# madsjulia/GeostatInversion.jl

Hardware: AMD Instinct MI355X
Metric: randSVD GB/s + top-k singular-value rel-err, n=1e6 rank=256 (higher is better)
Workload: dtype f64

## Files before the change

### geostatinversion.jl_amd/build.py

```python
import os
import shutil
import subprocess
import sys
from concurrent.futures import ThreadPoolExecutor

HERE = os.path.dirname(os.path.abspath(__file__))
CSRC = os.path.join(HERE, "csrc")
OBJ = os.path.join(HERE, "build")
LIB = os.path.join(HERE, "libgsi_hip.so")
SOURCES = ["gemm_f64.hip", "gemm_f64_gen1.hip", "syrk_f64.hip", "panel_lu_leaf.hip", "panel_lu_blocks.hip", "panel_lu_streamed.hip", "panel_lu_sharded.hip", "panel_qr.hip", "cholqr.hip", "lowrank_power.hip", "jacobi_svd.hip", "misc.hip", "lsqr_dev.hip", "pointcov_gemm.hip", "fft_cov.hip", "fft_gridcov_plan.hip", "fftrf_sample.hip",
           "hip_backend.hip", "pipeline.cpp", "api.cpp"]
HEADERS = ["backend.hpp", "hip_common.hpp", "panel_lu_dev.hpp", "pipeline.hpp", "lsqr_state.hpp", "pointcov.hpp", "pointcov_gen.hpp", "host_staging.hpp", "gemm_f64_kernel.inc.hpp", "fft_line.hpp", "jacobi_sched.hpp", "../../include/gsi_hip.h"]
CXXFLAGS = ["-O3", "-std=c++17", "-fPIC", "--offload-arch=gfx950", "-Wall", "-Wno-unused-function",
            "-Wno-unused-result", "-Wno-unused-value"]
RESOURCE_FLAG = "-Rpass-analysis=kernel-resource-usage"
_RES_KEYS = {"TotalSGPRs": "sgprs", "VGPRs": "vgprs", "AGPRs": "agprs", "ScratchSize [bytes/lane]": "scratch_bytes_per_lane",
             "Occupancy [waves/SIMD]": "occupancy_waves_per_simd", "SGPRs Spill": "sgpr_spills", "VGPRs Spill": "vgpr_spills",
             "LDS Size [bytes/block]": "lds_bytes_per_block", "Dynamic Stack": "dynamic_stack"}


def parse_resource_remarks(text):
    out, cur = {}, None
    for line in text.splitlines():
        if "remark:" not in line or "[-Rpass-analysis=kernel-resource-usage]" not in line:
            continue
        body = line.split("remark:", 1)[1].replace("[-Rpass-analysis=kernel-resource-usage]", "").strip()
        if ":" not in body:
            continue
        key, val = [x.strip() for x in body.rsplit(":", 1)]
        if key == "Function Name":
            cur = out.setdefault(val, {})
        elif cur is not None and key in _RES_KEYS:
            cur[_RES_KEYS[key]] = (val == "True") if key == "Dynamic Stack" else int(val)
    return out


def hipcc_version():
    r = subprocess.run([_hipcc(), "--version"], capture_output=True, text=True)
    lines = [ln.strip() for ln in r.stdout.splitlines() if ln.strip()]
    return "; ".join(lines[:2])


def kernel_resources():
# ... 74 lines not shown
```

### geostatinversion.jl_amd/context.py

```python
import ctypes as C

import numpy as np

from . import _lib as L


class Context:

    def __init__(self, device=0, lib=None):
        self.lib = lib or L.load()
        h = C.c_void_p()
        L.check(self.lib.gsi_ctx_create(C.byref(h), int(device)), self.lib)
        self.h = h
        self.device = int(device)
        self._children = []

    def close(self):
        if getattr(self, "h", None):
            for ch in list(self._children):
                ch.close()
            self.lib.gsi_ctx_destroy(self.h)
            self.h = None

    def __del__(self):
# ... 24 lines not shown
        out = np.empty((self.rank()[1], v.size))
        L.check(self.lib.gsi_ctx_host_allgather(self.h, L.dptr(v), v.size, L.dptr(out)), self.lib)
        return out

    def barrier(self):
        self.host_allgather([0.0])

    def shard(self, m):
        r, n = self.rank()
        pad = -(-m // n)
        row0 = min(r * pad, m)
        return row0, min(pad, m - row0)

    def profile(self, on=True):
        L.check(self.lib.gsi_ctx_profile(self.h, int(on)), self.lib)

    def phase_reset(self):
        L.check(self.lib.gsi_ctx_phase_reset(self.h), self.lib)

    def phase_times(self):
        ms = (C.c_double * len(L.PHASES))()
        cnt = (C.c_int64 * len(L.PHASES))()
        L.check(self.lib.gsi_ctx_phase_times(self.h, ms, cnt), self.lib)
        return {name: (ms[i], cnt[i]) for i, name in enumerate(L.PHASES)}

    def counters(self):
        out = (C.c_int64 * 4)()
        L.check(self.lib.gsi_ctx_counters(self.h, out), self.lib)
        return {"cholqr2": out[0], "householder": out[1], "jacobi_sweeps": out[2], "scholqr3": out[3]}

    LU_FORMS = ["none", "replicated", "per-step", "persistent-1hop", "persistent-2hop", "persistent-ov"]

    def path_info(self):
        n = 18
        out = (C.c_int64 * n)()
        L.check(self.lib.gsi_ctx_path_info(self.h, out, n), self.lib)
        forms = {self.LU_FORMS[f]: int(out[6 + f]) for f in range(1, 6) if out[6 + f]}
        return {"lu_form": self.LU_FORMS[out[0]] if 0 <= out[0] < 6 else int(out[0]), "lu_forms_run": forms,
                "lu_selftest_mask": int(out[1]), "collectives": int(out[2]), "n_ranks_seen": int(out[3]),
                "lu_timeouts": int(out[4]), "lu_timeouts_recovered": int(out[5]), "svd_sweep_cap_hits": int(out[12]),
                "lowrank_tails": int(out[13]), "lowrank_power_steps": int(out[14]), "lowrank_power_declines": int(out[15]),
                "lowrank_split_lus": int(out[16]), "lowrank_split_declines": int(out[17])}

    def release_cache(self):
        L.check(self.lib.gsi_ctx_release_cache(self.h), self.lib)

    def device_bytes(self):
        b = C.c_int64()
        L.check(self.lib.gsi_ctx_device_bytes(self.h, C.byref(b)), self.lib)
        return b.value


class _Handle:
    _destroy = None

    def __init__(self, ctx, h):
        self.ctx, self.h = ctx, h
        ctx._children.append(self)

    def close(self):
        if getattr(self, "h", None):
            getattr(self.ctx.lib, self._destroy)(self.h)
            self.h = None
            if self in self.ctx._children:
                self.ctx._children.remove(self)

    def __del__(self):
        try:
            self.close()
        except Exception:
            pass


class Operator(_Handle):
    _destroy = "gsi_op_destroy"
# ... 162 lines not shown
```

### geostatinversion.jl_amd/csrc/api.cpp

```cpp
#include <cmath>
#include <cstdlib>
#include <cstring>
#include <memory>
#include <new>
#include <string>
#include <vector>
#include "../../include/gsi_hip.h"
#include "pipeline.hpp"
#include "pointcov.hpp"

using namespace gsi;

struct gsi_ctx {
  Context c;
};
struct gsi_op {
  Operator op;
};
struct gsi_mat {
  gsi_ctx* ctx;
  Buf buf;
  int64_t rows, cols;
  int refs = 1;
};
// ... 135 lines not shown
    c.be->sync();
    if (!c.comm) {
      std::memcpy(all_out, mine, sizeof(double) * (size_t)count);
      return;
    }
    const int G = c.nranks();
    Buf send(c.be.get(), (size_t)count), recv(c.be.get(), (size_t)count * G);
    c.be->upload2d(send.p, count, mine, count, count, 1);
    const int64_t before = c.comm->ncollectives;
    c.comm->allgather(send.p, recv.p, (size_t)count);
    c.comm->ncollectives = before;
    c.be->download2d(all_out, count, recv.p, count, count, G);
  });
}

int gsi_ctx_path_info(gsi_ctx* ctx, int64_t* out, int64_t n_out) {
  return guarded([&] {
    REQUIRE(ctx && out && n_out >= 1, "bad argument");
    Context& c = ctx->c;
    int64_t v[GSI_PATH_INFO_COUNT] = {0};
    v[GSI_PATH_LU_FORM_LAST] = c.lu_form_last;
    v[GSI_PATH_LU_SELFTEST_MASK] = c.lus_mr_selftest;
    v[GSI_PATH_COLLECTIVES] = c.comm ? c.comm->ncollectives : 0;
    v[GSI_PATH_RANKS_SEEN] = c.ranks_seen;
    v[GSI_PATH_LU_TIMEOUTS] = c.be->lu_timeouts();
    v[GSI_PATH_LU_TIMEOUTS_RECOVERED] = c.lu_timeouts_recovered;
    for (int f = 0; f < (int)Context::LU_FORMS; ++f) v[GSI_PATH_LU_FORM_COUNTS + f] = c.lu_form_count[f];
    v[GSI_PATH_SVD_CAP_HITS] = c.be->svd_cap_hits();
    v[GSI_PATH_LOWRANK_TAILS] = c.lowrank_tails;
    v[GSI_PATH_LOWRANK_POWER_STEPS] = c.lowrank_power_steps;
    v[GSI_PATH_LOWRANK_POWER_DECLINES] = c.lowrank_power_declines;
    v[GSI_PATH_LOWRANK_SPLIT_LUS] = c.lowrank_split_lus;
    v[GSI_PATH_LOWRANK_SPLIT_DECLINES] = c.lowrank_split_declines;
    for (int64_t i = 0; i < n_out; ++i) out[i] = i < GSI_PATH_INFO_COUNT ? v[i] : 0;
  });
}

int gsi_ctx_pinned_copy_rate(gsi_ctx* ctx, int64_t bytes, double* h2d_gbs, double* d2h_gbs) {
  return guarded([&] {
    REQUIRE(ctx && h2d_gbs && d2h_gbs, "NULL argument");
    REQUIRE(bytes >= 0 && bytes <= ((int64_t)64 << 30), "bad size");
    ctx->c.be->pinned_copy_rate(bytes, h2d_gbs, d2h_gbs);
  });
}

int gsi_ctx_rank(gsi_ctx* ctx, int* rank, int* nranks) {
  return guarded([&] {
    REQUIRE(ctx, "ctx is NULL");
    if (rank) *rank = ctx->c.rank();
    if (nranks) *nranks = ctx->c.nranks();
  });
}

int gsi_op_dense(gsi_ctx* ctx, gsi_op** op, const double* A_rows, int64_t m, int64_t n, int64_t lda,
                 int64_t row0, int64_t m_local) {
  return guarded([&] {
    REQUIRE(ctx && op && A_rows, "NULL argument");
    *op = nullptr;
    REQUIRE(m >= 1 && n >= 1 && lda >= m_local && lda >= 1, "bad matrix shape");
    check_shard(ctx->c, m, row0, m_local);
    std::unique_ptr<gsi_op> o(new gsi_op());
    Operator& A = o->op;
    A.ctx = &ctx->c; A.kind = OP_DENSE; A.m = m; A.n = n; A.row0 = row0; A.mloc = m_local;
    A.ld = m_local > 0 ? ((m_local + 15) / 16) * 16 : 16;
    A.data = Buf(ctx->c.be.get(), (size_t)A.ld * n);
    ctx->c.be->upload2d(A.data.p, A.ld, A_rows, lda, m_local, n);
// ... 1035 lines not shown
```

### geostatinversion.jl_amd/csrc/backend.hpp

```cpp
#pragma once
#include <cstddef>
#include <cstdint>
#include <stdexcept>
#include <string>

namespace gsi {

struct Error : std::runtime_error {
  int code;
  Error(int c, const std::string& msg) : std::runtime_error(msg), code(c) {}
};

enum Phase : int {
  PH_GEMM_N = 0, PH_GEMM_T = 1, PH_LU = 2, PH_QR = 3, PH_SVD = 4, PH_SMALL_GEMM = 5,
  PH_COMM = 6, PH_OTHER = 7, PH_COMM_WAIT = 8, PH_COUNT = 9
};

class Backend {
 public:
  virtual ~Backend() {}
  virtual const char* name() const = 0;

  virtual double* alloc(size_t count) = 0;
  virtual void release(double* p) = 0;
// ... 153 lines not shown
                           double* out) = 0;

  virtual void gemv_n(int64_t m, int64_t k, double alpha, const double* A, int64_t lda, const double* x, double beta,
                      double* y) = 0;
  virtual void gemv_t(int64_t m, int64_t k, double alpha, const double* A, int64_t lda, const double* x, double* y) = 0;
  virtual void project_out(int64_t m, int64_t ncols, const double* q, double* Y, int64_t ld) = 0;
  virtual void scal(int64_t n, double a, double* x) = 0;
  virtual void diag_mul_add(int64_t n, const double* d, const double* x, double* y) = 0;

  virtual size_t lsqr_work_doubles() = 0;
  virtual void lsqr_begin(int64_t n, const double* w, double* work) = 0;
  virtual void lsqr_step_u(int64_t m, const double* t, double* u, double* work) = 0;
  virtual void lsqr_step_v(int64_t n, const double* t, double* v, double* w, double* x, double* work) = 0;

  virtual void f64_to_f32(const double* src, void* dst32, size_t count) = 0;
  virtual void pcga_params_f32(const void* Z32, int64_t n, int64_t K, const double* s, const double* X, double delta,
                               double* out) = 0;
  virtual void basis_gemv_f32(const void* Z32, int64_t n, int64_t K, const double* w, double beta, const double* X,
                              double* y) = 0;

  virtual int take_error(std::string* msg) = 0;
  virtual bool retryable_failure() { return false; }
  virtual void forgive_lost_coresidency() {}

  virtual void profile(bool on) = 0;
  virtual void phase_begin(Phase p) = 0;
  virtual void phase_end(Phase p) = 0;
  virtual void phase_end_more(Phase p) { phase_end(p); }
  virtual void phase_reset() = 0;
  virtual void phase_times(double* ms, int64_t* counts) = 0;
  virtual void counters(int64_t* out4) { out4[0] = out4[1] = out4[2] = out4[3] = 0; }
  virtual int64_t lu_timeouts() { return 0; }
  virtual int64_t svd_cap_hits() { return 0; }
  virtual void set_ranks_sharing_device(int n) { (void)n; }
};

class Comm {
 public:
  int rank = 0, nranks = 1;
  int64_t ncollectives = 0;
  virtual ~Comm() {}
  void allreduce_sum(double* buf, size_t count) { ++ncollectives; do_allreduce_sum(buf, count); }
  void allgather(const double* send, double* recv, size_t count) { ++ncollectives; do_allgather(send, recv, count); }
  void reduce_scatter_sum(const double* send, double* recv, size_t count) { ++ncollectives; do_reduce_scatter_sum(send, recv, count); }
  void alltoall(const double* send, double* recv, size_t count) { ++ncollectives; do_alltoall(send, recv, count); }
  virtual bool share_pointers(void* mine, size_t bytes, void** all) { (void)mine; (void)bytes; (void)all; return false; }
  virtual int ranks_on_my_device() { return 1; }
  virtual void host_barrier() {}

 protected:
  virtual void do_allreduce_sum(double* buf, size_t count) = 0;
  virtual void do_allgather(const double* send, double* recv, size_t count) = 0;
  virtual void do_reduce_scatter_sum(const double* send, double* recv, size_t count) = 0;
  virtual void do_alltoall(const double* send, double* recv, size_t count) = 0;
};

Backend* make_backend(int device_id);
Comm* make_comm(Backend* be, int nranks, int rank, const void* unique_id);
void comm_unique_id(void* id_out);
const char* backend_name();

struct ScopedPhase {
  Backend* be; Phase p;
  ScopedPhase(Backend* b, Phase ph) : be(b), p(ph) { be->phase_begin(p); }
  ~ScopedPhase() { be->phase_end(p); }
};
// ... 8 lines not shown
```

### geostatinversion.jl_amd/csrc/gemm_f64.hip

```cpp
#include <hip/hip_runtime.h>
#include <cstdint>
#include <cstdlib>
#include <type_traits>
#include <algorithm>
#include "hip_common.hpp"
#include "pointcov.hpp"
#include "pointcov_gen.hpp"

namespace gsi { namespace hipk {

#define GSI_GEMM_TILE_COUNTERS_32 1
#include "gemm_f64_kernel.inc.hpp"
void gemm_dispatch_gen1(int nt, dim3 grid, hipStream_t st, int64_t M, int64_t L, int64_t K, const double* A, int64_t lda,
                        const double* B, int64_t ldb, double* C, int64_t ldc, double alpha, double beta, double* slabs,
                        int64_t kchunk, int nchunks_x, int wide, int xmode, int tri, const GenA& gen, int64_t nitems);

__global__ void splitk_reduce_kernel(int64_t M, int64_t L, int nsplit, const double* __restrict__ slabs,
                                     double* __restrict__ C, int64_t ldc, double alpha, double beta) {
  const int64_t total = M * L;
  for (int64_t idx = (int64_t)blockIdx.x * blockDim.x + threadIdx.x; idx < total;
       idx += (int64_t)gridDim.x * blockDim.x) {
    double s = 0.0;
    for (int sp = 0; sp < nsplit; ++sp) s += slabs[(int64_t)sp * total + idx];
    const int64_t r = idx % M, c = idx / M;
    double v = alpha * s;
    if (beta != 0.0) v += beta * C[r + c * ldc];
    C[r + c * ldc] = v;
  }
}

int gemm_choose_split(int64_t nwg, int64_t K) {
  constexpr int64_t CUS = 256;
  static const bool legacy = getenv("GSI_GEMM_SPLIT_LEGACY") != nullptr;
  static const int forced = getenv("GSI_GEMM_FORCE_SPLIT") ? atoi(getenv("GSI_GEMM_FORCE_SPLIT")) : 0;
  if (forced > 0 && nwg >= 256 && K >= 64 * BK) return forced;
  if (legacy) {
    if (nwg >= 192 || K < 8 * BK) return 1;
    int64_t want = (CUS + nwg - 1) / nwg, cap = K / (4 * BK);
    if (want > cap) want = cap;
    return (int)(want < 1 ? 1 : (want > 64 ? 64 : want));
  }
  if (K < 8 * BK || nwg >= 16 * CUS) return 1;
  int64_t maxs = K / (4 * BK);
  if (maxs > 256) maxs = 256;
  int best = 1;
  double best_cost = (double)((nwg + CUS - 1) / CUS);
  for (int64_t s = 2; s <= maxs; ++s) {
    const double cost = (double)((nwg * s + CUS - 1) / CUS) / (double)s * (1.0 + 0.004 * (double)s);
// ... 34 lines not shown
  const int ntmax = gemm_chunk_tiles(tri);
  const int64_t nchunks = (tiles + ntmax - 1) / ntmax;
  const int nt = (int)((tiles + nchunks - 1) / nchunks);
  const int64_t rowblocks = (M + BMT - 1) / BMT;
  int64_t active = rowblocks * nchunks;
  if (tri == 1) {
    active = 0;
    for (int64_t rb = 0; rb < rowblocks; ++rb)
      for (int64_t cb = 0; cb < nchunks; ++cb)
        if (cb >= (rb * BMT) / ((int64_t)nt * 16)) ++active;
  }
  const int nsplit = (force_nsplit > 0) ? force_nsplit : ((K > 0) ? gemm_choose_split(active, K) : 1);
  int64_t kchunk = (K + nsplit - 1) / nsplit;
  kchunk = ((kchunk + BK - 1) / BK) * BK;
  if (kchunk == 0) kchunk = BK;
  const int ns_eff = (K > 0) ? (int)((K + kchunk - 1) / kchunk) : 1;
  dim3 grid((unsigned)active, (unsigned)ns_eff, 1);
  double* slabs = (ns_eff > 1) ? ws : nullptr;
  static const int ncus = [] { int dev = 0, n = 256; hipDeviceProp_t pr; if (hipGetDevice(&dev) == hipSuccess && hipGetDeviceProperties(&pr, dev) == hipSuccess) n = pr.multiProcessorCount; return n; }();
  static const bool persist_on = !(getenv("GSI_GEMM_PERSIST") != nullptr && getenv("GSI_GEMM_PERSIST")[0] == '0');
  int64_t nitems = 0;
  const bool a_ok = ((uintptr_t)A & 15) == 0 && (lda & 1) == 0;
  const bool b_ok = ((uintptr_t)B & 15) == 0 && (ldb & 1) == 0;
  const bool irregular_x = a_ok && (!b_ok || L % ((int64_t)nt * 16) != 0);
  const int wide = a_ok ? 1 : 0;
  const int xmode = big ? 2 : (irregular_x ? 1 : 0);
  if (persist_on && gen == nullptr && xmode == 0 && tri == 0 && ns_eff == 1 && (ncus & 7) == 0 && active >= 2 * (int64_t)ncus &&
      K <= 128 * BK) {
    nitems = active;
    grid.x = (unsigned)ncus;
  }
  if (plan != nullptr) *plan = {nt, nchunks, xmode, wide, ns_eff, nitems > 0 ? 1 : 0, (int64_t)grid.x, active};
  const GenA none = {nullptr, 1, 0, 0, 0, 0.0, 0.0, 0.0};
  if (gen != nullptr && gen_mode == 2)
    launch_dispatch<false, 2>(nt, grid, st, M, L, K, A, lda, B, ldb, C, ldc, alpha, beta, slabs, kchunk, (int)nchunks, wide, xmode, tri, *gen, nitems);
  else if (gen != nullptr)
    gemm_dispatch_gen1(nt, grid, st, M, L, K, A, lda, B, ldb, C, ldc, alpha, beta, slabs, kchunk, (int)nchunks, wide, xmode, tri, *gen, nitems);
  else if (transA)
    launch_dispatch<true, 0>(nt, grid, st, M, L, K, A, lda, B, ldb, C, ldc, alpha, beta, slabs, kchunk, (int)nchunks, wide, xmode, tri, none, nitems);
  else
    launch_dispatch<false, 0>(nt, grid, st, M, L, K, A, lda, B, ldb, C, ldc, alpha, beta, slabs, kchunk, (int)nchunks, wide, xmode, tri, none, nitems);
  if (ns_eff > 1) {
    const int64_t total = M * L;
    int blocks = (int)((total + 255) / 256);
    if (blocks > 2048) blocks = 2048;
    hipLaunchKernelGGL(splitk_reduce_kernel, dim3(blocks), dim3(256), 0, st, M, L, ns_eff, slabs, C, ldc,
                       alpha, beta);
  }
}

void gemm_splitk_reduce(hipStream_t st, int64_t M, int64_t L, int nsplit, const double* slabs, double* C, int64_t ldc) {
  const int64_t total = M * L;
  int blocks = (int)((total + 255) / 256);
  if (blocks > 2048) blocks = 2048;
  hipLaunchKernelGGL(splitk_reduce_kernel, dim3(blocks), dim3(256), 0, st, M, L, nsplit, slabs, C, ldc, 1.0, 0.0);
}

void gemm_f64(hipStream_t st, bool transA, int64_t M, int64_t L, int64_t K, double alpha, const double* A,
              int64_t lda, const double* B, int64_t ldb, double beta, double* C, int64_t ldc, double* ws, GemmPlan* plan) {
  gemm_launch(st, transA, nullptr, M, L, K, alpha, A, lda, B, ldb, beta, C, ldc, ws, 0, 1, 0, plan);
}

int gemm_split_for(int64_t M, int64_t L, int64_t K) {
  if (M <= 0 || L <= 0 || K <= 0) return 1;
  const int64_t tiles = (L + 15) / 16, nchunks = (tiles + NTMAX - 1) / NTMAX;
  const int64_t active = ((M + BMT - 1) / BMT) * nchunks;
// ... 53 lines not shown
```

### geostatinversion.jl_amd/csrc/gemm_f64_kernel.inc.hpp

```cpp
typedef double double4_t __attribute__((ext_vector_type(4)));

constexpr int MT = 2;
constexpr int BMT = 4 * 16 * MT;
constexpr int NTHREADS = 512;
constexpr int BK = 32;
constexpr int BKP = BK + 2;
constexpr int BMP = BMT + 16;
constexpr int NTMAX = 10;
constexpr int NSETS = 2;
constexpr int A_PAIRS = BMT * BK / (2 * NTHREADS);
constexpr int KSTEP_NN = 2 * NTHREADS / BMT;
constexpr int RSTEP = 2 * NTHREADS / BK;
static_assert(A_PAIRS * 2 * NTHREADS == BMT * BK, "tile does not divide over the threads");

struct GenA {
  const double* t2;
  int32_t ny;
  int32_t kind;
  int64_t roff;
  int64_t koff;
  double inv_ell2, sigma2, nugget;
  int32_t dim;
};

template <int NT, bool TRANS_A, int GEN, int XMODE>
__global__ __launch_bounds__(NTHREADS) void gemm_f64_kernel(
    int64_t M, int64_t L, int64_t K, const double* __restrict__ A, int64_t lda,
    const double* __restrict__ B, int64_t ldb, double* __restrict__ C, int64_t ldc, double alpha,
    double beta, double* __restrict__ slabs, int64_t kchunk, int nchunks_x, int wide, int tri, GenA gen, int64_t nitems) {
  static_assert(!(GEN != 0 && TRANS_A), "the generated operand is symmetric: only the NN form exists");
  constexpr bool CANP = (GEN == 0 && XMODE == 0);
  const bool persist = CANP && nitems > 0;
  constexpr bool RAGGED = XMODE != 0;
  constexpr bool BIG = XMODE == 2;
  using off_t = typename std::conditional<BIG, uint64_t, uint32_t>::type;
  constexpr int A_ELEMS = TRANS_A ? BMT * BKP : BK * BMP;
  constexpr int B_ELEMS = NT * 16 * BKP;
  constexpr int BUF_ELEMS = A_ELEMS + B_ELEMS;
  extern __shared__ double smem[];
  constexpr int LDS0 = (GEN == 2) ? 64 : 0;

  const int tid = threadIdx.x;
  const int lane = tid & 63;
  const int wave = tid >> 6;
  const int rg = wave & 3;
  const int ch = wave >> 2;
  constexpr int NTW = (NT + 1) / 2;
  const int jl = lane & 15;
  const int kk = lane >> 4;
  int64_t tile_lin = blockIdx.x;
  int split = (int)blockIdx.y;
  int64_t r0 = 0, c0 = 0;
  auto locate = [&](int64_t bx) __attribute__((always_inline)) {
    tile_lin = bx;
    const int T = (int)gridDim.x, S = (int)gridDim.y;
    if (S > 1 && (S & 7) == 0) {
      const int lin = (int)bx + T * (int)blockIdx.y;
      const int xcd = lin & 7, j = lin >> 3;
      split = xcd + 8 * (j / T);
      tile_lin = j % T;
    } else if (S == 1 && tri != 1 && nchunks_x > 1) {
      const int C8 = 8 * nchunks_x;
      const int nrb = (int)((M + BMT - 1) / BMT);
// ... 161 lines not shown
        }
        return;
      }
#pragma unroll
      for (int it = 0; it < B_PAIRS; ++it)
        if (!B_RAGGED || b_c + RSTEP * it < NT * 16)
          b_reg[set][it] = *reinterpret_cast<const double2*>(Bb + (b_off0 + (off_t)it * b_step));
      return;
    }
    if constexpr (GEN == 0) {
#pragma unroll
    for (int it = 0; it < A_PAIRS; ++it) {
      const char* p = Ab + (a_off0 + (off_t)it * a_step);
      const int64_t r = TRANS_A ? r0 + a_r + RSTEP * it : r0 + a_r;
      const int64_t k = TRANS_A ? k0 + a_k : k0 + a_k + KSTEP_NN * it;
      const bool ok0 = (r < M && k < kend);
      const bool ok1 = TRANS_A ? (r < M && k + 1 < kend) : (r + 1 < M && k < kend);
      a_reg[set][it].x = ok0 ? *reinterpret_cast<const double*>(p) : 0.0;
      a_reg[set][it].y = ok1 ? *reinterpret_cast<const double*>(p + 8) : 0.0;
    }
    }
#pragma unroll
    for (int it = 0; it < B_PAIRS; ++it) {
      const char* p = Bb + (b_off0 + (off_t)it * b_step);
      const int cl = b_c + RSTEP * it;
      const int64_t c = c0 + cl;
      const int64_t k = k0 + b_k;
      const bool okc = (cl < NT * 16) && (c < L);
      b_reg[set][it].x = (okc && k < kend) ? *reinterpret_cast<const double*>(p) : 0.0;
      b_reg[set][it].y = (okc && k + 1 < kend) ? *reinterpret_cast<const double*>(p + 8) : 0.0;
    }
  };

  auto stage = [&](int buf, auto SET, int64_t k0) __attribute__((always_inline)) {
    constexpr int set = decltype(SET)::value;
    double* a_s = smem + LDS0 + buf * BUF_ELEMS;
    double* b_s = a_s + A_ELEMS;
    (void)k0;
    if constexpr (GEN == 2) {
      const int kw = __builtin_amdgcn_readfirstlane(a_k);
      const int64_t row_first = gen.roff + r0;
      const int krem = (kend - k0 < BK) ? (int)(kend - k0) : BK;
#pragma unroll
      for (int it = 0; it < A_PAIRS; ++it) {
        const int64_t kc = k0 + kw + KSTEP_NN * it;
        const bool okk = kw + KSTEP_NN * it < krem;
        const int64_t gj = gen.koff + (okk ? kc : kbeg);
        const int64_t gju = ((int64_t)__builtin_amdgcn_readfirstlane((int)(gj >> 32)) << 32) |
                            (uint32_t)__builtin_amdgcn_readfirstlane((int)(gj & 0xffffffff));
        const double qx = A[4 * gju], qy = A[4 * gju + 1];
        double dx = p0x - qx, dy = p0y - qy;
        double s0 = fma(dx, dx, dy * dy);
        dx = p1x - qx; dy = p1y - qy;
        double s1 = fma(dx, dx, dy * dy);
        const int fl = gen_flags(gq.flags);
        if (fl & 1) {
          const double qz = A[4 * gju + 2];
          const double dz0 = p0z - qz, dz1 = p1z - qz;
          s0 = fma(dz0, dz0, s0); s1 = fma(dz1, dz1, s1);
        }
        double2 pr;
        gen_point_pair(gq, fl, s0, s1, gtab, pr.x, pr.y);
        const int rel = (int)(gju - row_first);
        if ((unsigned)rel < (unsigned)BMT) {
          pr.x += (a_r == rel) ? gen.nugget : 0.0;
          pr.y += (a_r + 1 == rel) ? gen.nugget : 0.0;
        }
        *reinterpret_cast<double2*>(a_s + (a_k + KSTEP_NN * it) * BMP + a_r) = pr;
      }
    } else
    if (TRANS_A) {
#pragma unroll
      for (int it = 0; it < A_PAIRS; ++it)
        *reinterpret_cast<double2*>(a_s + (a_r + RSTEP * it) * BKP + a_k) = a_reg[set][it];
    } else {
#pragma unroll
      for (int it = 0; it < A_PAIRS; ++it)
        *reinterpret_cast<double2*>(a_s + (a_k + KSTEP_NN * it) * BMP + a_r) = a_reg[set][it];
    }
#pragma unroll
    for (int it = 0; it < B_PAIRS; ++it)
      if (!B_RAGGED || b_c + RSTEP * it < NT * 16)
        *reinterpret_cast<double2*>(b_s + (b_c + RSTEP * it) * BKP + b_k) = b_reg[set][it];
  };

  double fa[MT], fan[MT];
  double fb[NTW];
  const int t0 = ch * NTW;
  const int ntw = (NT - t0 < NTW) ? ((NT - t0 > 0) ? NT - t0 : 0) : NTW;
  auto a_frag = [&](int buf, int s, int h) -> double {
    const double* a_s = smem + LDS0 + buf * BUF_ELEMS;
    return TRANS_A ? a_s[(16 * MT * rg + 16 * h + jl) * BKP + 4 * s + kk]
                   : a_s[(4 * s + kk) * BMP + 16 * MT * rg + 16 * h + jl];
  };
  auto b_frag = [&](int buf, int s, int t) -> double {
    const double* b_s = smem + LDS0 + buf * BUF_ELEMS + A_ELEMS;
    return b_s[(16 * (t0 + t) + jl) * BKP + 4 * s + kk];
  };

  using Set0 = std::integral_constant<int, 0>;
  using Set1 = std::integral_constant<int, 1>;
#if GSI_GEMM_TILE_COUNTERS_32
  auto do_tile = [&](int t, auto PAR) __attribute__((always_inline)) {
#else
  auto do_tile = [&](int64_t t, auto PAR) __attribute__((always_inline)) {
#endif
    constexpr int cur = decltype(PAR)::value;
    using NextSet = std::integral_constant<int, (NSETS == 2) ? (cur ^ 1) : 0>;
    auto chores = [&]() __attribute__((always_inline)) {
      __builtin_amdgcn_s_setprio(0);
#if GSI_GEMM_TILE_COUNTERS_32
      if (t + 1 < ntiles) stage(cur ^ 1, NextSet{}, kbeg + (int64_t)(t + 1) * BK);
      if (t + 1 + NSETS < ntiles) prefetch(t + 1 + NSETS, NextSet{});
#else
      if (t + 1 < ntiles) stage(cur ^ 1, NextSet{}, kbeg + (t + 1) * BK);
      if (t + 1 + NSETS < ntiles) prefetch(kbeg + (t + 1 + NSETS) * BK, NextSet{});
#endif
      __builtin_amdgcn_s_setprio(1);
    };
#pragma unroll
    for (int s = 0; s < BK / 4; ++s) {
      if (s == 1 && ch == 0) chores();
      if (s == 1 + BK / 8 && ch != 0) chores();
      const bool last = (s + 1 == BK / 4);
      if (last) __syncthreads();
      const int nbuf = last ? (cur ^ 1) : cur;
      const int ns = last ? 0 : s + 1;
      const bool more = !last || (t + 1 < ntiles);
      if (more) {
#pragma unroll
        for (int h = 0; h < MT; ++h) fan[h] = a_frag(nbuf, ns, h);
      }
#pragma unroll
      for (int tt = 0; tt < NTW; ++tt) {
        if ((NT % 2 == 0) || tt < ntw) {
#pragma unroll
          for (int h = 0; h < MT; ++h)
            acc[h][tt] = __builtin_amdgcn_mfma_f64_16x16x4f64(fb[tt], fa[h], acc[h][tt], 0, 0, 0);
          if (more) fb[tt] = b_frag(nbuf, ns, tt);
        }
      }
#pragma unroll
      for (int h = 0; h < MT; ++h) fa[h] = fan[h];
    }
  };

  int64_t item = blockIdx.x;
  bool primed = false;
  for (;;) {
    if (ntiles > 0) {
      if (!primed) {
#if GSI_GEMM_TILE_COUNTERS_32
        prefetch(0, Set0{});
        if (NSETS == 2 && ntiles > 1) prefetch(1, Set1{});
#else
        prefetch(kbeg, Set0{});
        if (NSETS == 2 && ntiles > 1) prefetch(kbeg + BK, Set1{});
#endif
      }
      stage(0, Set0{}, kbeg);
#if GSI_GEMM_TILE_COUNTERS_32
      if (ntiles > NSETS) prefetch(NSETS, Set0{});
#else
      if (ntiles > NSETS) prefetch(kbeg + NSETS * BK, Set0{});
#endif
      __syncthreads();
#pragma unroll
      for (int h = 0; h < MT; ++h) fa[h] = a_frag(0, 0, h);
#pragma unroll
      for (int t = 0; t < NTW; ++t)
        if ((NT % 2 == 0) || t < ntw) fb[t] = b_frag(0, 0, t);
#if GSI_GEMM_TILE_COUNTERS_32
      int t = 0;
#else
      int64_t t = 0;
#endif
      for (; t + 1 < ntiles; t += 2) {
        do_tile(t, Set0{});
        do_tile(t + 1, Set1{});
      }
      if (t < ntiles) do_tile(t, Set0{});
    }
    const int64_t er0 = r0, ec0 = c0;
    bool more = false;
    if constexpr (CANP) {
      if (persist && item + (int64_t)gridDim.x < nitems) {
        more = true;
        item += gridDim.x;
        __syncthreads();
        locate(item);
        setup_item();
        if (ntiles > 0) {
#if GSI_GEMM_TILE_COUNTERS_32
          prefetch(0, Set0{});
          if (NSETS == 2 && ntiles > 1) prefetch(1, Set1{});
#else
          prefetch(kbeg, Set0{});
          if (NSETS == 2 && ntiles > 1) prefetch(kbeg + BK, Set1{});
#endif
        }
        primed = true;
      }
    }

#pragma unroll
    for (int h = 0; h < MT; ++h) {
      const int64_t row = er0 + 16 * MT * rg + 16 * h + jl;
      if (row < M) {
        double* W = (slabs != nullptr) ? slabs + (int64_t)split * M * L : nullptr;
#pragma unroll
        for (int t = 0; t < NTW; ++t) {
          if ((NT % 2 == 0) || t < ntw) {
#pragma unroll
            for (int reg = 0; reg < 4; ++reg) {
              const int64_t col = ec0 + 16 * (t0 + t) + kk + 4 * reg;
              if (col < L) {
                if (W != nullptr) {
                  W[row + col * M] = acc[h][t][reg];
                } else {
                  double v = alpha * acc[h][t][reg];
                  if (beta != 0.0) v += beta * C[row + col * ldc];
                  C[row + col * ldc] = v;
                }
              }
            }
          }
        }
      }
    }
    if (!more) break;
#pragma unroll
    for (int h = 0; h < MT; ++h)
#pragma unroll
      for (int t = 0; t < NTW; ++t) acc[h][t] = (double4_t){0.0, 0.0, 0.0, 0.0};
  }
}

template <int NT, bool TRANS_A, int GEN, int XMODE>
static void launch_nt(dim3 grid, hipStream_t st, int64_t M, int64_t L, int64_t K, const double* A,
                      int64_t lda, const double* B, int64_t ldb, double* C, int64_t ldc, double alpha,
                      double beta, double* slabs, int64_t kchunk, int nchunks_x, int wide, int tri, const GenA& gen, int64_t nitems) {
  constexpr size_t shmem = 2 * ((TRANS_A ? BMT * BKP : BK * BMP) + NT * 16 * BKP) * sizeof(double) + (GEN == 2 ? 64 * sizeof(double) : 0);
  static std::atomic<uint64_t> attr_mask{0};
  if (first_use_on_this_device(attr_mask))
    (void)hipFuncSetAttribute((const void*)gemm_f64_kernel<NT, TRANS_A, GEN, XMODE>,
                              hipFuncAttributeMaxDynamicSharedMemorySize, (int)shmem);
  hipLaunchKernelGGL((gemm_f64_kernel<NT, TRANS_A, GEN, XMODE>), grid, dim3(NTHREADS), shmem, st, M, L, K, A, lda, B, ldb, C,
                     ldc, alpha, beta, slabs, kchunk, nchunks_x, wide, tri, gen, nitems);
}

template <bool TRANS_A, int GEN>
static void launch_dispatch(int nt, dim3 grid, hipStream_t st, int64_t M, int64_t L, int64_t K,
                            const double* A, int64_t lda, const double* B, int64_t ldb, double* C,
                            int64_t ldc, double alpha, double beta, double* slabs, int64_t kchunk, int nchunks_x, int wide,
                            int xmode, int tri, const GenA& gen, int64_t nitems) {
#define GSI_CASE(N)                                                                             \
  case N:                                                                                       \
    if (xmode == 2)                                                                               \
      launch_nt<N, TRANS_A, GEN, 2>(grid, st, M, L, K, A, lda, B, ldb, C, ldc, alpha, beta, slabs, kchunk, nchunks_x, wide, tri, gen, nitems); \
    else if (xmode == 1)                                                                          \
      launch_nt<N, TRANS_A, GEN, 1>(grid, st, M, L, K, A, lda, B, ldb, C, ldc, alpha, beta, slabs, kchunk, nchunks_x, wide, tri, gen, nitems); \
    else                                                                                          \
      launch_nt<N, TRANS_A, GEN, 0>(grid, st, M, L, K, A, lda, B, ldb, C, ldc, alpha, beta, slabs, kchunk, nchunks_x, wide, tri, gen, nitems); \
    break;
  switch (nt) {
#ifdef GSI_GEMM_DEV_ONLY_NT10
    GSI_CASE(10)
#else
    GSI_CASE(1) GSI_CASE(2) GSI_CASE(3) GSI_CASE(4) GSI_CASE(5)
    GSI_CASE(6) GSI_CASE(7) GSI_CASE(8) GSI_CASE(9) GSI_CASE(10)
#endif
    default: break;
  }
#undef GSI_CASE
}
```

### geostatinversion.jl_amd/csrc/hip_backend.hip

```cpp
#include <hip/hip_runtime.h>
#include <rccl/rccl.h>
#include <dlfcn.h>
#include <fcntl.h>
#include <sched.h>
#include <sys/mman.h>
#include <time.h>
#include <unistd.h>
#include <algorithm>
#include <cmath>
#include <cstdlib>
#include <cstring>
#include <condition_variable>
#include <atomic>
#include <mutex>
#include <string>
#include <chrono>
#include <map>
#include <memory>
#include <set>
#include <vector>
#include "../../include/gsi_hip.h"
#include "backend.hpp"
#include "hip_common.hpp"
#include "host_staging.hpp"
// ... 1342 lines not shown
  void phase_end_more(Phase) override { phase_end_counted(false); }
  void phase_end_counted(bool counted) {
    if (!prof_) return;
    if (roctx().pop) roctx().pop();
    hipEventRecord(cur_.b, st_);
    cur_.counted = counted;
    records_.push_back(cur_);
  }
  void phase_reset() override {
    bind();
    hipStreamSynchronize(st_);
    for (auto& r : records_) { ev_pool_.push_back(r.a); ev_pool_.push_back(r.b); }
    records_.clear();
    for (int i = 0; i < PH_COUNT; ++i) { acc_ms_[i] = 0.0; acc_n_[i] = 0; }
  }
  void phase_times(double* ms, int64_t* counts) override {
    bind();
    hipStreamSynchronize(st_);
    for (auto& r : records_) {
      float t = 0.f;
      if (hipEventElapsedTime(&t, r.a, r.b) == hipSuccess) { acc_ms_[r.phase] += t; acc_n_[r.phase] += r.counted ? 1 : 0; }
      ev_pool_.push_back(r.a);
      ev_pool_.push_back(r.b);
    }
    records_.clear();
    for (int i = 0; i < PH_COUNT; ++i) { ms[i] = acc_ms_[i]; counts[i] = acc_n_[i]; }
  }

  void counters(int64_t* out4) override {
    out4[0] = n_cholqr_; out4[1] = n_householder_; out4[2] = last_svd_sweeps_; out4[3] = n_scholqr3_;
  }
  int64_t lu_timeouts() override { return n_lu_timeouts_; }
  int64_t svd_cap_hits() override { return n_svd_cap_hits_; }
  void set_ranks_sharing_device(int n) override { ranks_sharing_device_ = n; }
  int device() const { return device_; }

 private:
  struct Scratch {
    HipBackend* be; double* p;
    Scratch(HipBackend* b, size_t doubles) : be(b), p(doubles ? b->alloc(doubles) : nullptr) {}
    ~Scratch() { if (p) be->release(p); }
    Scratch(const Scratch&) = delete;
    Scratch& operator=(const Scratch&) = delete;
  };
  struct Rec { Phase phase; hipEvent_t a, b; bool counted; };
  hipEvent_t get_event() {
    if (!ev_pool_.empty()) { hipEvent_t e = ev_pool_.back(); ev_pool_.pop_back(); return e; }
    hipEvent_t e;
    hipEventCreate(&e);
    return e;
  }
  void check_launch(const char* what) {
    hipError_t e = hipGetLastError();
    if (e != hipSuccess) throw Error(GSI_ERR_HIP, std::string(what) + ": " + hipGetErrorString(e));
  }
  void free_ws(DevBuf& b) {
    if (!b.p) return;
    if (b.pooled) release((double*)b.p);
    else { std::lock_guard<std::mutex> g(mu_); garbage_.push_back(b.p); garbage_bytes_ += b.bytes; }
    b.p = nullptr; b.bytes = 0; b.pooled = false;
  }
  void collect_garbage() {
    std::vector<void*> g;
    { std::lock_guard<std::mutex> lk(mu_); g.swap(garbage_); garbage_bytes_ = 0; }
    for (void* p : g) (void)hipFree(p);
  }
// ... 533 lines not shown
```

### geostatinversion.jl_amd/csrc/hip_common.hpp

```cpp
#pragma once
#include <hip/hip_runtime.h>
#include <atomic>
#include <cstdint>
#include <cstddef>
#include "pointcov.hpp"

namespace gsi { namespace hipk {

inline bool first_use_on_this_device(std::atomic<uint64_t>& mask) {
  int dev = 0;
  if (hipGetDevice(&dev) != hipSuccess || dev < 0 || dev > 63) return true;
  const uint64_t bit = (uint64_t)1 << dev;
  return (mask.fetch_or(bit, std::memory_order_acq_rel) & bit) == 0;
}

struct GemmPlan { int64_t nt, nchunks, xmode, wide, nsplit, persistent, grid_x, active; };
size_t gemm_workspace_doubles(int64_t M, int64_t L, int64_t K);
void gemm_f64(hipStream_t st, bool transA, int64_t M, int64_t L, int64_t K, double alpha, const double* A,
              int64_t lda, const double* B, int64_t ldb, double beta, double* C, int64_t ldc, double* ws,
              GemmPlan* plan = nullptr);
size_t gemm_rowblock_workspace_doubles(int64_t M_full, int64_t mb, int64_t L, int64_t K);
void gemm_f64_nn_rowblock(hipStream_t st, int64_t M_full, int64_t r0, int64_t mb, int64_t L, int64_t K, const double* A,
                          int64_t lda, const double* B, int64_t ldb, double* C, int64_t ldc, double* ws,
                          GemmPlan* plan = nullptr);
size_t gemm_syrk_workspace_doubles(int64_t l, int64_t m);
size_t syrk_upper_workspace_doubles(int64_t l, int64_t m);
bool syrk_full_from_upper(hipStream_t st, int64_t l, int64_t m, const double* Y, int64_t ld, double* G, int64_t ldg, double* ws);
bool trmm_upper_tall(hipStream_t st, int64_t m, int64_t l, const double* A, int64_t lda, const double* X, int64_t ldx, double* C,
                     int64_t ldc);
void gemm_f64_syrk_upper(hipStream_t st, int64_t l, int64_t m, const double* A, int64_t lda, double* C, int64_t ldc,
                         double* ws, GemmPlan* plan = nullptr);
void gemm_f64_trmm_upper(hipStream_t st, int64_t M, int64_t L, int64_t K, const double* A, int64_t lda, const double* B,
                         int64_t ldb, double* C, int64_t ldc, double* ws, GemmPlan* plan = nullptr);
void gemm_f64_gridcov(hipStream_t st, int64_t M, int64_t L, int64_t K, const double* tab, int64_t nx, int64_t ny,
                      int64_t roff, int64_t koff, const double* B, int64_t ldb, double* C, int64_t ldc, double* ws);

void gemm_f64_pointcov(hipStream_t st, int64_t M, int64_t L, int64_t K, const double* pts4, int64_t npts, int d, int kind,
                       double sigma2, double nugget, int64_t roff, int64_t koff, const double* B, int64_t ldb, double* C,
                       int64_t ldc, double* ws, double* xpack);
double pointcov_point_scale(int kind, double inv_ell);
bool gemm_f64_pointcov_wide(hipStream_t st, int64_t M, int64_t L, int64_t K, const double* pts4, int64_t npts, int d, int kind,
                            double sigma2, double nugget, int64_t roff, int64_t koff, const double* B, int64_t ldb, double* C,
                            int64_t ldc, double* ws, double* xpack);
size_t gemm_pointcov_workspace_doubles(int64_t M, int64_t L, int64_t K);
size_t gemm_pointcov_pack_doubles(int64_t M, int64_t L, int64_t K);
int gemm_choose_split(int64_t nwg, int64_t K);
void gemm_splitk_reduce(hipStream_t st, int64_t M, int64_t L, int nsplit, const double* slabs, double* C, int64_t ldc);
void pointcov_pad_points(hipStream_t st, const double* pts, int d, int64_t n, double scale, double* out4);
int64_t fft_embed_size(int64_t N);
size_t fft_plan_doubles(const int64_t M[3]);
// ... 179 lines not shown
```

### include/gsi_hip.h

```cpp
#ifndef GSI_HIP_H
#define GSI_HIP_H

#include <stdint.h>

#ifdef __cplusplus
extern "C" {
#endif

#define GSI_VERSION 100

#define GSI_OK 0
#define GSI_ERR_ARG 1
#define GSI_ERR_NEG_ITERS 2
#define GSI_ERR_SINGULAR 3
#define GSI_ERR_HIP 4
#define GSI_ERR_RCCL 5
#define GSI_ERR_OOM 6
#define GSI_ERR_NOT_POSDEF 7
#define GSI_ERR_INTERNAL 8

typedef struct gsi_ctx gsi_ctx;
typedef struct gsi_op gsi_op;
typedef struct gsi_mat gsi_mat;

// ... 128 lines not shown
                          double* out);
int gsi_pcga_update_basis(gsi_ctx* ctx, const gsi_basis* basis, const double* X, double beta_bar, const double* etas,
                          int64_t nobs, const double* xi_bar, double* s_out);
int gsi_basis_download_col(gsi_ctx* ctx, const gsi_basis* basis, int64_t col, double* host);

#define GSI_PHASE_GEMM_N 0
#define GSI_PHASE_GEMM_T 1
#define GSI_PHASE_LU 2
#define GSI_PHASE_QR 3
#define GSI_PHASE_SVD 4
#define GSI_PHASE_SMALL_GEMM 5
#define GSI_PHASE_COMM 6
#define GSI_PHASE_OTHER 7
#define GSI_PHASE_COMM_WAIT 8
#define GSI_NUM_PHASES 9
int gsi_ctx_profile(gsi_ctx* ctx, int enable);
int gsi_ctx_phase_reset(gsi_ctx* ctx);
int gsi_ctx_phase_times(gsi_ctx* ctx, double* ms_out ,
                        int64_t* count_out );
int gsi_ctx_counters(gsi_ctx* ctx, int64_t* out4);
#define GSI_PATH_LU_FORM_LAST 0
#define GSI_PATH_LU_SELFTEST_MASK 1
#define GSI_PATH_COLLECTIVES 2
#define GSI_PATH_RANKS_SEEN 3
#define GSI_PATH_LU_TIMEOUTS 4
#define GSI_PATH_LU_TIMEOUTS_RECOVERED 5
#define GSI_PATH_LU_FORM_COUNTS 6
#define GSI_PATH_SVD_CAP_HITS 12
#define GSI_PATH_LOWRANK_TAILS 13
#define GSI_PATH_LOWRANK_POWER_STEPS 14
#define GSI_PATH_LOWRANK_POWER_DECLINES 15
#define GSI_PATH_LOWRANK_SPLIT_LUS 16
#define GSI_PATH_LOWRANK_SPLIT_DECLINES 17
#define GSI_PATH_INFO_COUNT 18
int gsi_ctx_path_info(gsi_ctx* ctx, int64_t* out, int64_t n_out);
int gsi_ctx_pinned_copy_rate(gsi_ctx* ctx, int64_t bytes, double* h2d_gbs, double* d2h_gbs);
int gsi_ctx_release_cache(gsi_ctx* ctx);
int gsi_ctx_device_bytes(gsi_ctx* ctx, int64_t* bytes);

#ifdef __cplusplus
}
#endif
#endif
```

Measured before the change: 1653.

## Add streaming persistent NN GEMM variant that overlaps next-item prefetch with current tile

Adds a separately compiled streaming variant of the persistent f64 GEMM kernel for the stored NN wide NT=10 case with an even tile count. Blocks start loading the next work item's tiles during the last tiles of the current item, so the pipeline does not drain and re-prime between items. LDS addressing moves to byte offsets that advance incrementally to cut address arithmetic. It is on by default (GSI_GEMM_STREAM=0 disables it) and adds a launch counter to path_info. The cost is more code complexity and a risk of register pressure or correctness problems at item boundaries.

```diff
diff --git a/geostatinversion.jl_amd/build.py b/geostatinversion.jl_amd/build.py
--- a/geostatinversion.jl_amd/build.py
+++ b/geostatinversion.jl_amd/build.py
@@ -8,7 +8,7 @@
 CSRC = os.path.join(HERE, "csrc")
 OBJ = os.path.join(HERE, "build")
 LIB = os.path.join(HERE, "libgsi_hip.so")
-SOURCES = ["gemm_f64.hip", "gemm_f64_gen1.hip", "syrk_f64.hip", "panel_lu_leaf.hip", "panel_lu_blocks.hip", "panel_lu_streamed.hip", "panel_lu_sharded.hip", "panel_qr.hip", "cholqr.hip", "lowrank_power.hip", "jacobi_svd.hip", "misc.hip", "lsqr_dev.hip", "pointcov_gemm.hip", "fft_cov.hip", "fft_gridcov_plan.hip", "fftrf_sample.hip",
+SOURCES = ["gemm_f64.hip", "gemm_f64_gen1.hip", "gemm_f64_stream.hip", "syrk_f64.hip", "panel_lu_leaf.hip", "panel_lu_blocks.hip", "panel_lu_streamed.hip", "panel_lu_sharded.hip", "panel_qr.hip", "cholqr.hip", "lowrank_power.hip", "jacobi_svd.hip", "misc.hip", "lsqr_dev.hip", "pointcov_gemm.hip", "fft_cov.hip", "fft_gridcov_plan.hip", "fftrf_sample.hip",
            "hip_backend.hip", "pipeline.cpp", "api.cpp"]
 HEADERS = ["backend.hpp", "hip_common.hpp", "panel_lu_dev.hpp", "pipeline.hpp", "lsqr_state.hpp", "pointcov.hpp", "pointcov_gen.hpp", "host_staging.hpp", "gemm_f64_kernel.inc.hpp", "fft_line.hpp", "jacobi_sched.hpp", "../../include/gsi_hip.h"]
 CXXFLAGS = ["-O3", "-std=c++17", "-fPIC", "--offload-arch=gfx950", "-Wall", "-Wno-unused-function",
diff --git a/geostatinversion.jl_amd/context.py b/geostatinversion.jl_amd/context.py
--- a/geostatinversion.jl_amd/context.py
+++ b/geostatinversion.jl_amd/context.py
@@ -80,7 +80,7 @@
     LU_FORMS = ["none", "replicated", "per-step", "persistent-1hop", "persistent-2hop", "persistent-ov"]
 
     def path_info(self):
-        n = 18
+        n = 19
         out = (C.c_int64 * n)()
         L.check(self.lib.gsi_ctx_path_info(self.h, out, n), self.lib)
         forms = {self.LU_FORMS[f]: int(out[6 + f]) for f in range(1, 6) if out[6 + f]}
@@ -88,7 +88,8 @@
                 "lu_selftest_mask": int(out[1]), "collectives": int(out[2]), "n_ranks_seen": int(out[3]),
                 "lu_timeouts": int(out[4]), "lu_timeouts_recovered": int(out[5]), "svd_sweep_cap_hits": int(out[12]),
                 "lowrank_tails": int(out[13]), "lowrank_power_steps": int(out[14]), "lowrank_power_declines": int(out[15]),
-                "lowrank_split_lus": int(out[16]), "lowrank_split_declines": int(out[17])}
+                "lowrank_split_lus": int(out[16]), "lowrank_split_declines": int(out[17]),
+                "gemm_stream_launches": int(out[18])}
 
     def release_cache(self):
         L.check(self.lib.gsi_ctx_release_cache(self.h), self.lib)
diff --git a/geostatinversion.jl_amd/csrc/api.cpp b/geostatinversion.jl_amd/csrc/api.cpp
--- a/geostatinversion.jl_amd/csrc/api.cpp
+++ b/geostatinversion.jl_amd/csrc/api.cpp
@@ -191,6 +191,7 @@
     v[GSI_PATH_LOWRANK_POWER_DECLINES] = c.lowrank_power_declines;
     v[GSI_PATH_LOWRANK_SPLIT_LUS] = c.lowrank_split_lus;
     v[GSI_PATH_LOWRANK_SPLIT_DECLINES] = c.lowrank_split_declines;
+    v[GSI_PATH_GEMM_STREAM_LAUNCHES] = c.be->gemm_stream_launches();
     for (int64_t i = 0; i < n_out; ++i) out[i] = i < GSI_PATH_INFO_COUNT ? v[i] : 0;
   });
 }
diff --git a/geostatinversion.jl_amd/csrc/backend.hpp b/geostatinversion.jl_amd/csrc/backend.hpp
--- a/geostatinversion.jl_amd/csrc/backend.hpp
+++ b/geostatinversion.jl_amd/csrc/backend.hpp
@@ -209,6 +209,7 @@
   virtual void counters(int64_t* out4) { out4[0] = out4[1] = out4[2] = out4[3] = 0; }
   virtual int64_t lu_timeouts() { return 0; }
   virtual int64_t svd_cap_hits() { return 0; }
+  virtual int64_t gemm_stream_launches() { return 0; }
   virtual void set_ranks_sharing_device(int n) { (void)n; }
 };
 
diff --git a/geostatinversion.jl_amd/csrc/gemm_f64.hip b/geostatinversion.jl_amd/csrc/gemm_f64.hip
--- a/geostatinversion.jl_amd/csrc/gemm_f64.hip
+++ b/geostatinversion.jl_amd/csrc/gemm_f64.hip
@@ -1,4 +1,5 @@
 #include <hip/hip_runtime.h>
+#include <atomic>
 #include <cstdint>
 #include <cstdlib>
 #include <type_traits>
@@ -14,6 +15,12 @@
 void gemm_dispatch_gen1(int nt, dim3 grid, hipStream_t st, int64_t M, int64_t L, int64_t K, const double* A, int64_t lda,
                         const double* B, int64_t ldb, double* C, int64_t ldc, double alpha, double beta, double* slabs,
                         int64_t kchunk, int nchunks_x, int wide, int xmode, int tri, const GenA& gen, int64_t nitems);
+
+void gemm_dispatch_stream(dim3 grid, hipStream_t st, int64_t M, int64_t L, int64_t K, const double* A, int64_t lda,
+                          const double* B, int64_t ldb, double* C, int64_t ldc, double alpha, double beta, int64_t kchunk,
+                          int nchunks_x, int64_t nitems);
+static std::atomic<int64_t> stream_launches{0};
+int64_t gemm_stream_launches() { return stream_launches.load(std::memory_order_relaxed); }
 
 __global__ void splitk_reduce_kernel(int64_t M, int64_t L, int nsplit, const double* __restrict__ slabs,
                                      double* __restrict__ C, int64_t ldc, double alpha, double beta) {
@@ -114,6 +121,13 @@
   }
   if (plan != nullptr) *plan = {nt, nchunks, xmode, wide, ns_eff, nitems > 0 ? 1 : 0, (int64_t)grid.x, active};
   const GenA none = {nullptr, 1, 0, 0, 0, 0.0, 0.0, 0.0};
+  static const bool stream_on = !(getenv("GSI_GEMM_STREAM") != nullptr && getenv("GSI_GEMM_STREAM")[0] == '0');
+  const int64_t ktiles = (K + BK - 1) / BK;
+  if (stream_on && nitems > 0 && !transA && wide != 0 && nt == 10 && ktiles >= 4 && (ktiles & 1) == 0) {
+    gemm_dispatch_stream(grid, st, M, L, K, A, lda, B, ldb, C, ldc, alpha, beta, kchunk, (int)nchunks, nitems);
+    stream_launches.fetch_add(1, std::memory_order_relaxed);
+    return;
+  }
   if (gen != nullptr && gen_mode == 2)
     launch_dispatch<false, 2>(nt, grid, st, M, L, K, A, lda, B, ldb, C, ldc, alpha, beta, slabs, kchunk, (int)nchunks, wide, xmode, tri, *gen, nitems);
   else if (gen != nullptr)
diff --git a/geostatinversion.jl_amd/csrc/gemm_f64_kernel.inc.hpp b/geostatinversion.jl_amd/csrc/gemm_f64_kernel.inc.hpp
--- a/geostatinversion.jl_amd/csrc/gemm_f64_kernel.inc.hpp
+++ b/geostatinversion.jl_amd/csrc/gemm_f64_kernel.inc.hpp
@@ -1,3 +1,11 @@
+#ifndef GSI_GEMM_STREAM
+#define GSI_GEMM_STREAM 0
+#endif
+#if GSI_GEMM_STREAM
+#define GSI_GEMM_KERNEL gemm_f64_stream_kernel
+#else
+#define GSI_GEMM_KERNEL gemm_f64_kernel
+#endif
 typedef double double4_t __attribute__((ext_vector_type(4)));
 
 constexpr int MT = 2;
@@ -24,11 +32,15 @@
 };
 
 template <int NT, bool TRANS_A, int GEN, int XMODE>
-__global__ __launch_bounds__(NTHREADS) void gemm_f64_kernel(
+__global__ __launch_bounds__(NTHREADS) void GSI_GEMM_KERNEL(
     int64_t M, int64_t L, int64_t K, const double* __restrict__ A, int64_t lda,
     const double* __restrict__ B, int64_t ldb, double* __restrict__ C, int64_t ldc, double alpha,
     double beta, double* __restrict__ slabs, int64_t kchunk, int nchunks_x, int wide, int tri, GenA gen, int64_t nitems) {
   static_assert(!(GEN != 0 && TRANS_A), "the generated operand is symmetric: only the NN form exists");
+#if GSI_GEMM_STREAM
+  static_assert(GEN == 0 && XMODE == 0 && !TRANS_A && GSI_GEMM_TILE_COUNTERS_32, "the streaming mode exists for the stored NN form only");
+  bool next_item = false;
+#endif
   constexpr bool CANP = (GEN == 0 && XMODE == 0);
   const bool persist = CANP && nitems > 0;
   constexpr bool RAGGED = XMODE != 0;
@@ -256,6 +268,27 @@
     }
   };
 
+#if GSI_GEMM_STREAM
+  constexpr uint32_t BUF_BYTES = 8u * BUF_ELEMS;
+  char* const lds = reinterpret_cast<char*>(smem);
+  uint32_t wa_off = 8u * (uint32_t)(LDS0 + a_k * BMP + a_r);
+  uint32_t wb_off = 8u * (uint32_t)(LDS0 + A_ELEMS + b_c * BKP + b_k);
+  uint32_t fa_off = 8u * (uint32_t)(LDS0 + kk * BMP + 16 * MT * rg + jl);
+  uint32_t fb_off = 8u * (uint32_t)(LDS0 + A_ELEMS + (16 * (ch * ((NT + 1) / 2)) + jl) * BKP + kk);
+  auto stage = [&](auto BUF, auto SET) __attribute__((always_inline)) {
+    constexpr int set = decltype(SET)::value;
+#pragma unroll
+    for (int it = 0; it < A_PAIRS; ++it)
+      *reinterpret_cast<double2*>(lds + wa_off + 8 * (KSTEP_NN * it) * BMP) = a_reg[set][it];
+#pragma unroll
+    for (int it = 0; it < B_PAIRS; ++it)
+      if (!B_RAGGED || b_c + RSTEP * it < NT * 16)
+        *reinterpret_cast<double2*>(lds + wb_off + 8 * (RSTEP * it) * BKP) = b_reg[set][it];
+    constexpr uint32_t d = decltype(BUF)::value == 0 ? BUF_BYTES : 0u - BUF_BYTES;
+    wa_off += d; wb_off += d;
+    asm volatile("" : "+v"(wa_off), "+v"(wb_off));
+  };
+#else
   auto stage = [&](int buf, auto SET, int64_t k0) __attribute__((always_inline)) {
     constexpr int set = decltype(SET)::value;
     double* a_s = smem + LDS0 + buf * BUF_ELEMS;
@@ -307,11 +340,20 @@
       if (!B_RAGGED || b_c + RSTEP * it < NT * 16)
         *reinterpret_cast<double2*>(b_s + (b_c + RSTEP * it) * BKP + b_k) = b_reg[set][it];
   };
+#endif
 
   double fa[MT], fan[MT];
   double fb[NTW];
   const int t0 = ch * NTW;
   const int ntw = (NT - t0 < NTW) ? ((NT - t0 > 0) ? NT - t0 : 0) : NTW;
+#if GSI_GEMM_STREAM
+  auto a_frag = [&](int, int s, int h) -> double {
+    return *reinterpret_cast<const double*>(lds + fa_off + 8 * (4 * s * BMP + 16 * h));
+  };
+  auto b_frag = [&](int, int s, int t) -> double {
+    return *reinterpret_cast<const double*>(lds + fb_off + 8 * (16 * t * BKP + 4 * s));
+  };
+#else
   auto a_frag = [&](int buf, int s, int h) -> double {
     const double* a_s = smem + LDS0 + buf * BUF_ELEMS;
     return TRANS_A ? a_s[(16 * MT * rg + 16 * h + jl) * BKP + 4 * s + kk]
@@ -321,6 +363,7 @@
     const double* b_s = smem + LDS0 + buf * BUF_ELEMS + A_ELEMS;
     return b_s[(16 * (t0 + t) + jl) * BKP + 4 * s + kk];
   };
+#endif
 
   using Set0 = std::integral_constant<int, 0>;
   using Set1 = std::integral_constant<int, 1>;
@@ -333,7 +376,11 @@
     using NextSet = std::integral_constant<int, (NSETS == 2) ? (cur ^ 1) : 0>;
     auto chores = [&]() __attribute__((always_inline)) {
       __builtin_amdgcn_s_setprio(0);
-#if GSI_GEMM_TILE_COUNTERS_32
+#if GSI_GEMM_STREAM
+      if (t + 1 < ntiles || next_item) stage(std::integral_constant<int, cur ^ 1>{}, NextSet{});
+      const int tp = t + 1 + NSETS;
+      if (tp < ntiles || next_item) prefetch(tp < ntiles ? tp : tp - ntiles, NextSet{});
+#elif GSI_GEMM_TILE_COUNTERS_32
       if (t + 1 < ntiles) stage(cur ^ 1, NextSet{}, kbeg + (int64_t)(t + 1) * BK);
       if (t + 1 + NSETS < ntiles) prefetch(t + 1 + NSETS, NextSet{});
 #else
@@ -348,9 +395,20 @@
       if (s == 1 + BK / 8 && ch != 0) chores();
       const bool last = (s + 1 == BK / 4);
       if (last) __syncthreads();
+#if GSI_GEMM_STREAM
+      if (last) {
+        constexpr uint32_t d = cur == 0 ? BUF_BYTES : 0u - BUF_BYTES;
+        fa_off += d; fb_off += d;
+        asm volatile("" : "+v"(fa_off), "+v"(fb_off));
+      }
+#endif
       const int nbuf = last ? (cur ^ 1) : cur;
       const int ns = last ? 0 : s + 1;
+#if GSI_GEMM_STREAM
+      const bool more = !last || (t + 1 < ntiles) || next_item;
+#else
       const bool more = !last || (t + 1 < ntiles);
+#endif
       if (more) {
 #pragma unroll
         for (int h = 0; h < MT; ++h) fan[h] = a_frag(nbuf, ns, h);
@@ -369,6 +427,34 @@
     }
   };
 
+#if GSI_GEMM_STREAM
+  (void)persist; (void)p0x; (void)p0y; (void)p0z; (void)p1x; (void)p1y; (void)p1z;
+  int64_t item = blockIdx.x;
+  bool primed = false;
+  for (;;) {
+    next_item = item + (int64_t)gridDim.x < nitems;
+    const int64_t er0 = r0, ec0 = c0;
+    if (!primed) {
+      prefetch(0, Set0{});
+      prefetch(1, Set1{});
+      stage(Set0{}, Set0{});
+      prefetch(NSETS, Set0{});
+      __syncthreads();
+#pragma unroll
+      for (int h = 0; h < MT; ++h) fa[h] = a_frag(0, 0, h);
+#pragma unroll
+      for (int t = 0; t < NTW; ++t)
+        if ((NT % 2 == 0) || t < ntw) fb[t] = b_frag(0, 0, t);
+    }
+    for (int t = 0; t + 1 < ntiles; t += 2) {
+      do_tile(t, Set0{});
+      if (t + 4 == ntiles && next_item) { item += gridDim.x; locate(item); setup_item(); }
+      do_tile(t + 1, Set1{});
+    }
+    const bool more = next_item;
+    primed = true;
+
+#else
   int64_t item = blockIdx.x;
   bool primed = false;
   for (;;) {
@@ -427,6 +513,33 @@
       }
     }
 
+#endif
+#if GSI_GEMM_STREAM
+#pragma unroll
+    for (int h = 0; h < MT; ++h) {
+      const int64_t row = er0 + 16 * MT * rg + 16 * h + jl;
+      if (row < M) {
+        int64_t col = ec0 + 16 * t0 + kk;
+        int64_t off = row + col * ldc;
+#pragma unroll
+        for (int t = 0; t < NTW; ++t) {
+          if ((NT % 2 == 0) || t < ntw) {
+#pragma unroll
+            for (int reg = 0; reg < 4; ++reg) {
+              if (col < L) {
+                double v = alpha * acc[h][t][reg];
+                if (beta != 0.0) v += beta * C[off];
+                C[off] = v;
+              }
+              col += 4;
+              off += 4 * ldc;
+              asm volatile("" : "+v"(off));
+            }
+          }
+        }
+      }
+    }
+#else
 #pragma unroll
     for (int h = 0; h < MT; ++h) {
       const int64_t row = er0 + 16 * MT * rg + 16 * h + jl;
@@ -452,6 +565,7 @@
         }
       }
     }
+#endif
     if (!more) break;
 #pragma unroll
     for (int h = 0; h < MT; ++h)
@@ -467,9 +581,9 @@
   constexpr size_t shmem = 2 * ((TRANS_A ? BMT * BKP : BK * BMP) + NT * 16 * BKP) * sizeof(double) + (GEN == 2 ? 64 * sizeof(double) : 0);
   static std::atomic<uint64_t> attr_mask{0};
   if (first_use_on_this_device(attr_mask))
-    (void)hipFuncSetAttribute((const void*)gemm_f64_kernel<NT, TRANS_A, GEN, XMODE>,
+    (void)hipFuncSetAttribute((const void*)GSI_GEMM_KERNEL<NT, TRANS_A, GEN, XMODE>,
                               hipFuncAttributeMaxDynamicSharedMemorySize, (int)shmem);
-  hipLaunchKernelGGL((gemm_f64_kernel<NT, TRANS_A, GEN, XMODE>), grid, dim3(NTHREADS), shmem, st, M, L, K, A, lda, B, ldb, C,
+  hipLaunchKernelGGL((GSI_GEMM_KERNEL<NT, TRANS_A, GEN, XMODE>), grid, dim3(NTHREADS), shmem, st, M, L, K, A, lda, B, ldb, C,
                      ldc, alpha, beta, slabs, kchunk, nchunks_x, wide, tri, gen, nitems);
 }
 
diff --git a/geostatinversion.jl_amd/csrc/gemm_f64_stream.hip b/geostatinversion.jl_amd/csrc/gemm_f64_stream.hip
--- /dev/null
+++ b/geostatinversion.jl_amd/csrc/gemm_f64_stream.hip
@@ -0,0 +1,24 @@
+#include <hip/hip_runtime.h>
+#include <atomic>
+#include <cstdint>
+#include <cstdlib>
+#include <type_traits>
+#include <algorithm>
+#include "hip_common.hpp"
+#include "pointcov.hpp"
+#include "pointcov_gen.hpp"
+
+namespace gsi { namespace hipk {
+
+#define GSI_GEMM_TILE_COUNTERS_32 1
+#define GSI_GEMM_STREAM 1
+#include "gemm_f64_kernel.inc.hpp"
+
+void gemm_dispatch_stream(dim3 grid, hipStream_t st, int64_t M, int64_t L, int64_t K, const double* A, int64_t lda,
+                          const double* B, int64_t ldb, double* C, int64_t ldc, double alpha, double beta, int64_t kchunk,
+                          int nchunks_x, int64_t nitems) {
+  const GenA none = {nullptr, 1, 0, 0, 0, 0.0, 0.0, 0.0};
+  launch_nt<10, false, 0, 0>(grid, st, M, L, K, A, lda, B, ldb, C, ldc, alpha, beta, nullptr, kchunk, nchunks_x,  1,  0, none, nitems);
+}
+
+}}
diff --git a/geostatinversion.jl_amd/csrc/hip_backend.hip b/geostatinversion.jl_amd/csrc/hip_backend.hip
--- a/geostatinversion.jl_amd/csrc/hip_backend.hip
+++ b/geostatinversion.jl_amd/csrc/hip_backend.hip
@@ -1398,6 +1398,7 @@
   }
   int64_t lu_timeouts() override { return n_lu_timeouts_; }
   int64_t svd_cap_hits() override { return n_svd_cap_hits_; }
+  int64_t gemm_stream_launches() override { return hipk::gemm_stream_launches(); }
   void set_ranks_sharing_device(int n) override { ranks_sharing_device_ = n; }
   int device() const { return device_; }
 
diff --git a/geostatinversion.jl_amd/csrc/hip_common.hpp b/geostatinversion.jl_amd/csrc/hip_common.hpp
--- a/geostatinversion.jl_amd/csrc/hip_common.hpp
+++ b/geostatinversion.jl_amd/csrc/hip_common.hpp
@@ -16,6 +16,7 @@
 
 struct GemmPlan { int64_t nt, nchunks, xmode, wide, nsplit, persistent, grid_x, active; };
 size_t gemm_workspace_doubles(int64_t M, int64_t L, int64_t K);
+int64_t gemm_stream_launches();
 void gemm_f64(hipStream_t st, bool transA, int64_t M, int64_t L, int64_t K, double alpha, const double* A,
               int64_t lda, const double* B, int64_t ldb, double beta, double* C, int64_t ldc, double* ws,
               GemmPlan* plan = nullptr);
diff --git a/include/gsi_hip.h b/include/gsi_hip.h
--- a/include/gsi_hip.h
+++ b/include/gsi_hip.h
@@ -184,7 +184,8 @@
 #define GSI_PATH_LOWRANK_POWER_DECLINES 15
 #define GSI_PATH_LOWRANK_SPLIT_LUS 16
 #define GSI_PATH_LOWRANK_SPLIT_DECLINES 17
-#define GSI_PATH_INFO_COUNT 18
+#define GSI_PATH_GEMM_STREAM_LAUNCHES 18
+#define GSI_PATH_INFO_COUNT 19
 int gsi_ctx_path_info(gsi_ctx* ctx, int64_t* out, int64_t n_out);
 int gsi_ctx_pinned_copy_rate(gsi_ctx* ctx, int64_t bytes, double* h2d_gbs, double* d2h_gbs);
 int gsi_ctx_release_cache(gsi_ctx* ctx);
```

After: 1662, median of 6. No clear change (+0.6%).
